# ddiazdom/grlBWT

Measured on AMD Instinct MI355X. Metric: input MB/s building BCR BWT on 10 GB DNA reads, 1/2/4/8 MI355X, higher is better.
Workload: dtype u8; 1 GPU; 66225166 x 150 bp Illumina-style reads (10000000066 bytes) from a 330000000 bp genome, 0.5% substitutions; BASELINE configs[3]; input_resident=HBM, output=.rl_bwt image in HBM, parallelism=1 GPU

## Files before the change

### grlbwt_amd/csrc/capi_impl.hpp

```cpp
#include "../../include/grlbwt_hip.h"

#include <fcntl.h>
#include <zlib.h>
#include <sys/stat.h>
#include <unistd.h>

#include <atomic>
#include <chrono>
#include <cstdio>
#include <cstring>
#include <condition_variable>
#include <memory>
#include <mutex>
#include <string>
#include <system_error>
#include <thread>
#include <vector>


struct grlbwt_fm {
    uint32_t flags = 0;
    std::unique_ptr<grl32::Engine::FmIndex> f32;
    std::unique_ptr<grl64::Engine::FmIndex> f64;
};
// ... 1360 lines not shown
    for (uint64_t nbits : sizes)
        for (int kind = 0; kind < 5; kind++) {
            if (int rc = test_set_bits_one<uint32_t>(nbits, kind, seed + kind)) return -(500 + rc);
            if (int rc = test_set_bits_one<uint64_t>(nbits, kind, seed + 7 + kind)) return -(510 + rc);
        }
#ifdef GRLBWT_PRIM_HIP
    for (uint32_t span = 8; span <= 64; span <<= 1)
        for (int kind = 2; kind <= 4; kind += 2) {
            if (int rc = test_set_bits_one<uint32_t>(sizes[6], kind, seed + 20 + kind, span)) return -(520 + rc);
            if (int rc = test_set_bits_one<uint64_t>(sizes[5], kind, seed + 30 + kind, span)) return -(530 + rc);
        }
#endif
    return 0;
}

int selftest(uint64_t n, uint64_t seed) {
    if (n < 2) n = 2;
    std::vector<uint32_t> h(n);
    uint64_t s = seed;
    for (uint64_t i = 0; i < n; i++) h[i] = (uint32_t)sm64(s);
    grl32::DBuf<uint32_t> d(n);
    prim::h2d(d.p, h.data(), n * 4);
    {
        grl32::DBuf<uint64_t> o(n + 1);
        uint64_t tot = prim::exclusive_scan<uint64_t>(n, U32In{d.p}, o.p, true, "selftest.scan");
        auto ho = o.to_host(n + 1);
        uint64_t acc = 0;
        for (uint64_t i = 0; i < n; i++) { if (ho[i] != acc) return -1; acc += h[i] & 1023u; }
        if (ho[n] != acc || tot != acc) return -2;
    }
// ... 44 lines not shown
    { int r = test_sort<uint64_t, uint32_t>(n, seed + 8, 51); if (r) return -110 - r; }
    { int r = test_sort_keys(n, seed + 9, 18); if (r) return -120 - r; }
    { int r = test_sort<uint32_t, uint64_t>(n, seed + 10, 27); if (r) return -130 - r; }
    { int r = test_sort<uint32_t, uint32_t>(n, seed + 11, 20); if (r) return -140 - r; }
    { int r = test_part(n, seed + 12, 6); if (r) return -150 - r; }
    { int r = test_part(n, seed + 13, 11); if (r) return -160 - r; }
    { int r = test_part(n, seed + 14, 18); if (r) return -170 - r; }
    { int r = test_pair_scan<uint32_t, uint32_t>(n, h, d.p); if (r) return -70 - r; }
    { int r = test_pair_scan<uint64_t, uint64_t>(n, h, d.p); if (r) return -80 - r; }
    { int r = test_stream_merge(n, seed); if (r) return r; }
#ifdef GRLBWT_PRIM_HIP
    { int r = test_seg_sort_all(seed + 40); if (r) return r; }
#endif
    { int r = test_pack(); if (r) return r; }
    { int r = test_set_bits(n, seed + 60); if (r) return r; }
    return 0;
}

}

extern "C" {

int grlbwt_abi_version(void) { return GRLBWT_ABI_VERSION; }
const char *grlbwt_backend_name(void) { return prim::kIsDevice ? "hip-gfx950" : "serial-test-standin"; }

const char *grlbwt_strerror(int code) {
    switch (code) {
        case GRLBWT_OK: return "ok";
        case GRLBWT_EINVAL: return "invalid argument or call out of order";
        case GRLBWT_EDEVICE: return "HIP device/runtime error";
// ... 555 lines not shown
```

### grlbwt_amd/csrc/engine_impl.hpp

```cpp

#include "switches.hpp"

namespace GRL_NS {

using prim::u8;
using prim::u16;
using prim::u32;
using prim::u64;
typedef GRL_IDX_T idx_t;

template <class T>
struct DBuf {
    T *p = nullptr;
    u64 n = 0;
    DBuf() {}
    explicit DBuf(u64 n_) { alloc(n_); }
    DBuf(const DBuf &) = delete;
    DBuf &operator=(const DBuf &) = delete;
    DBuf(DBuf &&o) noexcept : p(o.p), n(o.n) { o.p = nullptr; o.n = 0; }
    DBuf &operator=(DBuf &&o) noexcept {
        if (this != &o) { release(); p = o.p; n = o.n; o.p = nullptr; o.n = 0; }
        return *this;
    }
    ~DBuf() { release(); }
// ... 14 lines not shown
}

template <class T>
GRL_HD u64 upper_bound(const T *a, u64 n, T v) {
    u64 lo = 0, hi = n;
    while (lo < hi) { u64 mid = (lo + hi) >> 1; if (a[mid] <= v) lo = mid + 1; else hi = mid; }
    return lo;
}
template <class T>
GRL_HD u64 lower_bound(const T *a, u64 n, T v) {
    u64 lo = 0, hi = n;
    while (lo < hi) { u64 mid = (lo + hi) >> 1; if (a[mid] < v) lo = mid + 1; else hi = mid; }
    return lo;
}

template <class cell_t, bool FIRST>
struct CellOps {
    cell_t sep;
    GRL_HD u32 sym(cell_t c) const { return FIRST ? (u32)c : (u32)(c >> 2); }
    GRL_HD bool rep(cell_t c) const { return FIRST ? true : (bool)((c >> 1) & 1); }
    GRL_HD bool isT(cell_t c) const { return FIRST ? (c == sep) : (bool)(c & 1); }
};

GRL_HD bool bit_at(const u64 *w, u64 i) { return (w[i >> 6] >> (i & 63)) & 1ull; }
GRL_HD u64 next_set_bit(const u64 *w, u64 p, u64 n) {
    u64 r = n;
    if (p < n) {
        u64 wi = p >> 6;
        u64 x = w[wi] >> (p & 63);
        if (x) r = p + (u64)__builtin_ctzll(x);
        else {
            bool found = false;
            for (wi++; !found && (wi << 6) < n; wi++) { x = w[wi]; if (x) { r = (wi << 6) + (u64)__builtin_ctzll(x); found = true; } }
// ... 52 lines not shown
    const u64 *w;
    GRL_DEV u64 operator()(u64 i) const { return (u64)__builtin_popcountll(w[i]); }
};
struct PopcIn32 {
    const u64 *w;
    GRL_DEV u32 operator()(u64 i) const { return (u32)__builtin_popcountll(w[i]); }
};

static constexpr u64 kPosBits = 40;
static constexpr u64 kPosMask = (1ull << kPosBits) - 1;
static constexpr u64 kLenSat = 4095;
static constexpr u64 kExactKey = 1ull << 63;
GRL_HD u64 key_len(u64 k) { return (k >> kPosBits) & 0xFFFull; }
GRL_HD bool key_lastT(u64 k) { return (k >> (kPosBits + 12)) & 1ull; }
GRL_HD u64 key_pos(u64 k) { return (k & kPosMask) - 1; }

struct PhraseHash {
    u32 a, b;
    GRL_HD static PhraseHash init() { return PhraseHash{0x85A308D3u, 0x243F6A88u}; }
    GRL_HD void add(u32 v) {
        a = (a ^ v) * 0x9E3779B1u;
        b = (b + v) * 0x85EBCA6Bu;
        b ^= b >> 15;
    }
    GRL_HD u64 finish(u64 len) const {
        u64 h = ((u64)a << 32) | (u64)b;
        h ^= len * 0xC2B2AE3D27D4EB4Full;
        h ^= h >> 33; h *= 0xFF51AFD7ED558CCDull; h ^= h >> 33; h *= 0xC4CEB9FE1A85EC53ull; h ^= h >> 29;
        return h;
    }
// ... 42 lines not shown
    u64 hot_mask = 0;
    u32 slot_base = 0;
    static constexpr u32 kDirectSlots = 1u << 22;
    u32 dir_on = 0, dir_b0 = 0, dir_b1 = 0, dir_b2 = 0;
    u64 *dir_rep = nullptr;
    GRL_DEV u32 direct_index(u64 chunk, u32 len) const {
        const u64 ones = 0x0101010101010101ull;
        const u64 c = ((chunk >> dir_b0) & ones) | (((chunk >> dir_b1) & ones) << 1) | (((chunk >> dir_b2) & ones) << 2);
        const u32 lo = (u32)c, hi = (u32)(c >> 32);
        const u32 plo = (lo & 7u) | ((lo >> 5) & 0x38u) | ((lo >> 10) & 0x1C0u) | ((lo >> 15) & 0xE00u);
        const u32 phi = (hi & 7u) | ((hi >> 5) & 0x38u) | ((hi >> 10) & 0x1C0u) | ((hi >> 15) & 0xE00u);
        const u32 top = 1u << (3u * len);
        return ((plo | (phi << 12)) & (top - 1u)) | top;
    }
    GRL_DEV void first_seen(u32 slot, u64 item) const { if (dir_on && slot < kDirectSlots) dir_rep[slot] = item; }
    u64 *rec_k = nullptr; u64 *rec_hi = nullptr; int rec_b = 0; u32 rec_cmax = 0;
    u32 *long_count = nullptr;
    u64 walk_cap = ~0ull;
    static constexpr bool kExact = FIRST && sizeof(cell_t) == 1;
#ifndef GRL_HASH_BATCH
#define GRL_HASH_BATCH 4
#endif
    static constexpr int kBatch = kExact ? GRL_HASH_BATCH : 1;
    static constexpr u64 kCh = 8 / sizeof(cell_t);
    GRL_DEV static u64 load8(const cell_t *a) { u64 v; __builtin_memcpy(&v, a, 8); return v; }
    GRL_DEV bool same_phrase(u64 q, u64 p, u64 len, bool check_bits) const {
        bool same = true;
        if (q + len > n) { scal[1] = 3; scal[2] = (u32)q; scal[3] = (u32)len; same = false; }
        if (same && check_bits) {
            const u64 nq = next_set_bit(startbits, q + 1, n);
// ... 38 lines not shown
                const u64 len = (u64)eo + 1;
                if (ord >= n_occ) { scal[1] = 5; scal[2] = (u32)p; scal[3] = (u32)ord; }
                else if (rec_k) {
                    const u64 hi = khi | (((tm >> eo) & 1u) ? kPhrLastT : 0ull) | (len << 61);
                    rec_k[ord] = rec_key(klo, hi);
                    rec_hi[ord] = hi;
                    out_slot[ord] = 0;
                }
                fast = true;
            }
        }
        u32 res = prim::kNoBucket;
        if (!fast) res = process_walk(p, ord, pack);
        return res;
    }
    u64 *giant_list = nullptr; u32 *giant_n = nullptr; u32 giant_cap = 0;
    static constexpr u64 kLongWalk = 4096;
    GRL_DEV void giant_bounds(u64 item, u64 &p, u64 &ee) const {
        p = item;
        const u64 ns = next_set_bit_far(startbits, p + 1, n);
        ee = (ns >= n || ops.isT(t[ns - 1])) ? ns - 1 : ns;
    }
    GRL_DEV u64 giant_piece(u64 p, u64 ee, int lane) const {
        const u64 len = ee - p + 1, piece = (len + 63) / 64;
        u64 x = p + (u64)lane * piece;
        const u64 xe = x + piece < ee + 1 ? x + piece : ee + 1;
        const u64 cnt = xe > x ? xe - x : 0;
        PhraseHash ph = PhraseHash::init();
        while (x + 4 * kCh <= xe) {
            u64 ck[4];
// ... 83 lines not shown
                ok = false;
            } else {
                if (long_count) prim::atomic_add(long_count, 1u);
                if (rec_k) { rec_k[ord] = ord; rec_hi[ord] = 0ull; }
            }
        }
        if (ok) {
            u64 len = e - p + 1;
            if (kExact && len <= 7) {
                u64 content = 0;
                for (u64 j = 0; j < len; j++) content |= (u64)t[p + j] << (8 * j);
                const u64 mine = kExactKey | (len << 60) | content;
                if (dir_on) found = direct_index(content, (u32)len);
                else
                found = insert_exact(mine, p, exact_hash(mine) & (hot_keys ? hot_mask : mask), 0, false);
            } else found = find_or_insert(p, len, use_giant ? PhraseHash{(u32)(*giant_acc >> 32), (u32)*giant_acc}.finish(len) : ph.finish(len), ops.isT(t[e]));
            if (found != prim::kNoBucket) out_slot[ord] = (found & ~prim::kClaimBit) | (pack ? kLongMark : 0u);
        }
        return found;
    }
    GRL_DEV void process_batch(const u64 *item, const bool *valid, u32 *slot) const { process_batch_exact<false>(item, valid, slot, nullptr, nullptr); }
    static constexpr bool kStream = kExact;
    GRL_DEV u64 ordinal_base(u64 p) const { return (u64)wordbase[p >> 6]; }
    GRL_DEV u64 next_item(u64 p) const {
        const u64 b0 = p + 1;
        u64 bits = startbits[b0 >> 6] >> (b0 & 63);
        if ((b0 & 63) > 56) bits |= startbits[(b0 >> 6) + 1] << (64 - (b0 & 63));
        bits &= 0xFFull;
        return bits ? b0 + (u64)__builtin_ctzll(bits) : p + 9;
    }
// ... 272 lines not shown
    const u64 *words; const u32 *base; u64 *pos;
    GRL_DEV void operator()(u64 w) const {
        u64 x = words[w];
        u64 k = base[w];
        while (x) { pos[k++] = w * 64 + (u64)__builtin_ctzll(x); x &= x - 1; }
    }
};
template <class F>
struct ListedFn {
    F f; const u64 *pos;
    static constexpr int kBatch = 1;
    static constexpr bool kClaims = F::kClaims;
    u64 *claim_bits = nullptr;
    GRL_DEV u64 claim_pos(u64 v) const { return pos[v]; }
    GRL_DEV bool is_start(u64) const { return true; }
    GRL_DEV u32 process(u64 v) const { return f.process(pos[v]); }
    GRL_DEV u32 operator()(u64 v) const { return f.process(pos[v]); }
    GRL_DEV void process_batch(const u64 *, const bool *, u32 *) const {}
    GRL_DEV void first_seen(u32 slot, u64 v) const { f.first_seen(slot, pos[v]); }
};

template <class cell_t, bool FIRST>
struct CompactTableFn {
    const cell_t *t;
    CellOps<cell_t, FIRST> ops;
    const u64 *startbits;
    const u64 *keys; const idx_t *counts;
    u64 *ph_pos; idx_t *ph_freq; u32 *ph_len; u32 *ph_slot; u8 *ph_lastT;
    int ks; u64 cs; const u64 *rep_pos;
    u64 n;
    GRL_DEV void emit(u64 s, u64 k) const {
        u64 k64 = keys[s << ks];
        u64 pos, len;
        bool lastT;
        if (k64 & kExactKey) {
            len = (k64 >> 60) & 7ull;
            pos = rep_pos[s];
            lastT = ops.isT((cell_t)(k64 >> (8 * (len - 1))));
        } else {
            pos = key_pos(k64); len = key_len(k64);
            lastT = key_lastT(k64);
            if (len == kLenSat) {
                const u64 ns = next_set_bit_far(startbits, pos + 1, n);
                const u64 e = (ns >= n || ops.isT(t[ns - 1])) ? ns - 1 : ns;
                len = e - pos + 1;
            }
        }
        ph_pos[k] = pos; ph_freq[k] = counts[s * cs]; ph_len[k] = (u32)len; ph_slot[k] = (u32)s;
        ph_lastT[k] = lastT ? 1 : 0;
    }
// ... 2297 lines not shown
        u64 Ds = 0; int part_bits = 0, rec_b = 0; u32 slot0 = 0;
        DBuf<prim::U128> ph_key;
        DBuf<u32> lid, pbase;
        DBuf<u8> ph_vflag;
        DBuf<u64> pstart;
        prim::RecSort psort;
        void clear() {
            n_occ = D = S = cap = Ds = 0; maxlen = 0; part_bits = rec_b = 0; slot0 = 0;
            next_text.release(); ph_pos.release(); ph_freq.release(); ph_len.release(); ph_slot.release(); ph_off.release(); ph_lastT.release();
            ph_key.release(); ph_vflag.release(); pstart.release(); lid.release(); pbase.release(); psort.release();
        }
    };

    struct PartPlan { bool on = false; int rec_b = 0; u32 rec_cmax = 0; int part_bits = 0; };
    struct SamplePlan { u64 blk = 0, stride = 0, n = 0, distinct = 0, long_occ = 0; double frac = 1.0; };
    struct TablePlan { u64 cap = 0, cap_max = 0, cap_hot = 0; bool aggregate = false, interleaved = false, direct = false; int ks = 0; u64 cs = 1; u32 dir_b[3] = {0, 0, 0}; u64 sym_of_code = 0; };
    static bool direct_index_bits(const u64 sym_present[4], u32 bits[3], u64 &sym_of_code) {
        int syms[256], ns = 0;
        for (int i = 0; i < 256; i++) if ((sym_present[i >> 6] >> (i & 63)) & 1ull) syms[ns++] = i;
        if (ns > 8) return false;
        for (u32 a = 0; a < 8; a++) for (u32 b = a + 1; b < 8; b++) for (u32 c = b + 1; c < 8; c++) {
            u32 seen = 0; bool ok = true; u64 soc = 0;
            for (int k = 0; k < ns && ok; k++) {
                const u32 code = ((syms[k] >> a) & 1u) | (((syms[k] >> b) & 1u) << 1) | (((syms[k] >> c) & 1u) << 2);
                if (seen & (1u << code)) ok = false;
                seen |= 1u << code;
                soc |= (u64)syms[k] << (8 * code);
            }
            if (ok) { bits[0] = a; bits[1] = b; bits[2] = c; sym_of_code = soc; return true; }
        }
        return false;
// ... 59 lines not shown
            if (part.on) want = (u64)(3.0 * (double)smp.long_occ * ((double)n / (double)n_s)) + 4096;
            tab.cap = 4096; while (tab.cap < want) tab.cap <<= 1;
            if (tab.cap > tab.cap_max) tab.cap = tab.cap_max;
            if (prim::sw().table_trace) fprintf(stderr, "[grlbwt] level %d: sample %llu occurrences, %llu distinct -> table %llu slots for %llu occurrences\n",
                                                      prim::rt().tag, (unsigned long long)occ_s, (unsigned long long)smp.distinct, (unsigned long long)tab.cap, (unsigned long long)n_occ);
        }
        void plan_table() {
            claim.alloc(nwords + 1);
            if (part.on) { rec_k.alloc(n_occ); rec_hi.alloc(n_occ); }
            const bool force_direct = HF::kExact && !part.on && prim::sw().force_direct_index;
            tab.aggregate = smp.frac < 0.25 || force_direct;
            tab.interleaved = !tab.aggregate;
            tab.ks = tab.interleaved ? 1 : 0; tab.cs = tab.interleaved ? 16 / sizeof(idx_t) : 1;
            if (HF::kExact && tab.aggregate && (smp.n || force_direct) && !part.on && E.sym_present_known && !prim::sw().no_direct_index)
                tab.direct = direct_index_bits(E.sym_present, tab.dir_b, tab.sym_of_code);
            if (tab.direct && (const void *)t == E.text0 && E.text0 != (const void *)E.own0.p) {
                if constexpr (sizeof(cell_t) == 1) {
                    const u64 stride = n >= (1ull << 22) ? n >> 20 : 1, m = n / stride;
                    const u64 foreign = prim::reduce_sum<u64>(m, ForeignByteIn{(const u8 *)t, stride, E.sym_present[0], E.sym_present[1], E.sym_present[2], E.sym_present[3]}, "hash_prepare");
                    if (foreign) throw prim::Error(-22, "the attached text has changed since its statistics were taken (a cell value that was not there)");
                }
            }
            const bool hot = !tab.direct && tab.aggregate && smp.n && !part.on && !prim::sw().no_hot_table;
            if (!tab.direct && !hot) return;
            if (tab.direct) tab.cap_hot = HF::kDirectSlots;
            else for (tab.cap_hot = 1024; tab.cap_hot < 4 * smp.distinct;) tab.cap_hot <<= 1;
            if (tab.cap_max > (1ull << 30)) tab.cap_max = 1ull << 30;
            if (tab.cap > tab.cap_max) tab.cap = tab.cap_max;
            if (!prim::sw().table_trace) return;
            if (tab.direct) fprintf(stderr, "[grlbwt] level %d: direct index on bits %u, %u, %u of a cell (%llu slots in front of the table)\n", prim::rt().tag,
// ... 2 lines not shown
                         (unsigned long long)tab.cap_hot, (unsigned long long)smp.distinct);
        }
        void alloc_table() {
            if (tab.interleaved) { keys.alloc(2 * tab.cap); keys.zero(); }
            else { keys.alloc(tab.cap_hot + tab.cap); counts.alloc(tab.cap_hot + tab.cap); keys.zero(); counts.zero(); }
            cnt = tab.interleaved ? (idx_t *)(keys.p + 1) : counts.p;
            if (HF::kExact) rep_pos.alloc(tab.cap_hot + tab.cap);
            scal.zero(); claim.zero();
        }
        void fill_hot_table(HF &f) {
            HF fh{t, ops, startbits.p, wordbase.p, keys.p, tab.cap_hot - 1, tab.cap_hot, 0, P.next_text.p, scal.p, n, n_occ, rep_pos.p, claim.p};
            fh.walk_cap = HF::kLongWalk;
            prim::for_each_agg(smp.n, SampledFn<HF>{fh, smp.blk, smp.stride, claim.p}, NoCountAdd{}, false, "hash_hot");
            f.hot_keys = keys.p; f.hot_mask = tab.cap_hot - 1; f.slot_base = (u32)tab.cap_hot;
        }
        void hash_listed(const HF &f, DBuf<u64> &lbits, bool aggregate) {
            DBuf<u32> lbase(nwords + 1);
            const u64 nl = (u64)prim::exclusive_scan<u32>(nwords, PopcIn32{lbits.p}, lbase.p, false, "hash_long_list");
            DBuf<u64> lpos(nl ? nl : 1);
            if (nl) prim::for_each(nwords, BitPositionsFn{lbits.p, lbase.p, lpos.p}, "hash_long_list");
            lbits.release(); lbase.release();
            if (nl) prim::for_each_agg(nl, ListedFn<HF>{f, lpos.p, claim.p}, SlotCountAdd{cnt, tab.cs}, aggregate, "hash_long_phrases");
        }
        void records_and_long_phrases(const HF &f) {
            prim::dev_memset(P.next_text.p, 0, n_occ * sizeof(u32));
            DBuf<u64> lbits(nwords + 1); lbits.zero();
            auto records = [&](auto bw) {
                prim::for_each_set_bit<idx_t>(n, startbits.p, wordbase.p, PhraseRecordFn<cell_t, decltype(bw)::value>{t, ops, startbits.p, wordbase.p, n, n_occ,
                                                                                                               rec_k.p, rec_hi.p, part.rec_b, part.rec_cmax, lbits.p, scal.p}, "hash_phrases");
            };
            switch (part.rec_b) {
#define GRL_REC_CASE(BW) case BW: records(std::integral_constant<int, BW>()); break;
                GRL_REC_CASE(10) GRL_REC_CASE(11) GRL_REC_CASE(12) GRL_REC_CASE(13) GRL_REC_CASE(14) GRL_REC_CASE(15) GRL_REC_CASE(16)
// ... 3 lines not shown
                default: records(std::integral_constant<int, 0>()); break;
            }
            hash_listed(f, lbits, false);
        }
        void name_stream_and_long_phrases(const HF &f) {
            DBuf<u64> lbits(nwords + 1); lbits.zero();
            prim::name_stream(n, f, SlotCountAdd{cnt, tab.cs}, lbits.p, "hash_phrases");
            hash_listed(f, lbits, tab.aggregate);
        }
        bool hash_pass() {
            alloc_table();
            HF f{t, ops, startbits.p, wordbase.p, keys.p + tab.cap_hot, tab.cap - 1, (tab.cap == tab.cap_max) ? tab.cap : 96 , tab.ks,
                 P.next_text.p, scal.p, n, n_occ, rep_pos.p ? rep_pos.p + tab.cap_hot : nullptr, claim.p};
            if (part.on) { f.rec_k = rec_k.p; f.rec_hi = rec_hi.p; f.rec_b = part.rec_b; f.rec_cmax = part.rec_cmax; }
            f.giant_list = giant_list.p; f.giant_n = scal.p + 4; f.giant_cap = (u32)std::min<u64>(giant_cap, 0xFFFFFFFFull);
            if (tab.direct) { f.dir_on = 1; f.dir_b0 = tab.dir_b[0]; f.dir_b1 = tab.dir_b[1]; f.dir_b2 = tab.dir_b[2]; f.dir_rep = rep_pos.p; f.slot_base = (u32)tab.cap_hot; }
            else if (tab.cap_hot) fill_hot_table(f);
            if constexpr (!FIRST) {
                if (part.on && !prim::sw().part_one_pass) records_and_long_phrases(f);
                else prim::for_each_agg(n, f, SlotCountAdd{cnt, tab.cs}, tab.aggregate, "hash_phrases");
            } else if (tab.direct && n_occ < 0xFFFFFFF0ull && !prim::sw().no_name_stream) name_stream_and_long_phrases(f);
            else prim::for_each_agg(n, f, SlotCountAdd{cnt, tab.cs}, tab.aggregate, "hash_phrases");
            std::vector<u32> sc = scal.to_host(8);
            if (sc[4] && !sc[1]) {
                prim::for_each_giant((u64)sc[4], giant_list.p, f, SlotCountAdd{cnt, tab.cs}, "hash_giant_phrases");
                sc = scal.to_host(8);
            }
            if (sc[1] == 1) return false;
            if (sc[1]) throw prim::Error(-71, "phrase hashing: consistency check " + std::to_string(sc[1]) + " failed (" +
                                                   std::to_string(sc[2]) + ", " + std::to_string(sc[3]) + ")");
            if (tab.direct) prim::for_each(tab.cap_hot, DirectFixFn{cnt, keys.p, rep_pos.p, claim.p, tab.sym_of_code}, "hash_direct_fix");
            P.cap = tab.cap_hot + tab.cap;
            return true;
        }
        bool dedupe_partitions() {
            StageTimer st(&E.tm.hash, "hash");
            DBuf<u64> rec_k2(n_occ), rec_hi2(n_occ);
            const int res = P.psort.forward(rec_k.p, rec_hi.p, rec_k2.p, rec_hi2.p, n_occ, part.part_bits, "phrase_part");
            DBuf<u64> skey, shi;
            if (res) { skey = std::move(rec_k2); shi = std::move(rec_hi2); dkey = std::move(rec_k); dhi = std::move(rec_hi); }
            else { skey = std::move(rec_k); shi = std::move(rec_hi); dkey = std::move(rec_k2); dhi = std::move(rec_hi2); }
            const u64 nparts = (u64)1 << part.part_bits;
            P.pstart.alloc(nparts + 1);
            prim::for_each(nparts + 1, prim::RecBoundsFn{skey.p, n_occ, part.part_bits, nparts, P.pstart.p}, "phrase_part.bounds");
            P.lid.alloc(n_occ); P.pbase.alloc(nparts + 1); dcnt.alloc(n_occ);
// ... 15 lines not shown
            StageTimer st(&E.tm.dict_sort, "dict_sort");
            DBuf<idx_t> cbase(nwords + 1);
            const u64 Dl = (u64)prim::exclusive_scan<idx_t>(nwords, PopcIn{claim.p}, cbase.p, false, "table_compact");
            const u64 D = Ds + Dl;
            if (D >= 0xFFFFFFF0ull) throw prim::Error(-75, "dictionary too large (>= 2^32 phrases)");
            P.D = D;
            P.ph_pos.alloc(D); P.ph_freq.alloc(D); P.ph_len.alloc(D); P.ph_slot.alloc(D); P.ph_lastT.alloc(D); P.ph_off.alloc(D + 1);
            if (part.on) {
                P.ph_key.alloc(Ds); P.ph_vflag.alloc(Ds);
                prim::for_each(((u64)1 << part.part_bits) * 64, PartPhraseFn{P.pbase.p, P.pstart.p, dkey.p, dhi.p, dcnt.p, P.slot0, P.ph_key.p, P.ph_pos.p, P.ph_freq.p,
                                                                          P.ph_len.p, P.ph_slot.p, P.ph_lastT.p, P.ph_vflag.p}, "phrase_dedupe.phrases");
                dkey.release(); dhi.release(); dcnt.release();
            }
            prim::for_each(nwords, ClaimSlotsFn{claim.p, cbase.p, startbits.p, wordbase.p, P.next_text.p, P.ph_slot.p + Ds}, "table_compact");
            prim::for_each(Dl, ClaimCompactFn<cell_t, FIRST>{CompactTableFn<cell_t, FIRST>{t, ops, startbits.p, keys.p, cnt, P.ph_pos.p + Ds,
                                                             P.ph_freq.p + Ds, P.ph_len.p + Ds, P.ph_slot.p + Ds, P.ph_lastT.p + Ds, tab.ks, tab.cs, rep_pos.p, n}}, "table_compact");
            wordbase.release(); claim.release();
            const prim::Pair<u64, u64> fl = prim::reduce_sum<prim::Pair<u64, u64>>(D, FreqLenIn{P.ph_freq.p, P.ph_len.p}, "dict_totals");
            if (fl.a != n_occ) throw prim::Error(-71, "phrase frequencies (" + std::to_string(fl.a) + ") do not add up to the parse size (" +
                                                           std::to_string(n_occ) + ")");
            P.maxlen = prim::reduce_max<u32>(D, LenIn{P.ph_len.p}, "dict_maxlen");
            if (fl.b >= 0xFFFFFFF0ull) throw prim::Error(-75, "dictionary too large (>= 2^32 symbols)");
            prim::exclusive_scan_nosync<u32>(D, LenIn{P.ph_len.p}, P.ph_off.p, true, "dict_offsets");
            P.S = fl.b;
        }
    };
    template <class cell_t, bool FIRST>
    void hash_local(const cell_t *t, u64 n, CellOps<cell_t, FIRST> ops, LocalParse &P, LevelData &L, bool allow_part = false) {
        for (;; allow_part = false, P.clear()) {
            NameStage<cell_t, FIRST> Z(*this, t, n, ops, P, L);
            Z.classify();
// ... 2263 lines not shown
```

### grlbwt_amd/csrc/prim_hip.hpp

```cpp
#pragma once
#include <hip/hip_runtime.h>
#include <cstdint>
#include <cstdio>
#include <cstdlib>
#include <cstring>
#include <chrono>
#include <stdexcept>
#include <string>
#include <vector>
#include <map>
#include <utility>
#include <type_traits>

#define GRLBWT_PRIM_HIP 1
#include "switches.hpp"

#define GRL_HD __host__ __device__ __forceinline__
#define GRL_DEV __device__ __forceinline__

namespace prim {

typedef uint8_t u8;
typedef uint16_t u16;
typedef uint32_t u32;
// ... 581 lines not shown
        unsigned long long m = __ballot(b);
        if ((threadIdx.x & 63) == 0) words[i >> 6] = m;
    }
}
template <class F>
inline void bitvector_from_pred(u64 n, F pred, u64 *words, const char *name = "bitvector") {
    if (n == 0) return;
    u64 n_padded = (n + 63) & ~u64(63);
    prof_begin(name);
    hipLaunchKernelGGL(k_bitvector<F>, dim3(grid_for(n_padded, kBlock)), dim3(kBlock), 0, rt().stream, n_padded, n,
                       pred, words);
    prof_end();
    after_launch(name);
}

template <class cell_t, class OPS>
__global__ void __launch_bounds__(kBlock) k_start_bits(u64 n, const cell_t *t, OPS ops, u64 *words) {
    constexpr int CPL = 16 / (int)sizeof(cell_t);
    constexpr int TILE = kBlock * CPL;
    constexpr int C = sizeof(cell_t) == 1 ? 8 : (sizeof(cell_t) == 8 ? 2 : 4);
    constexpr int WPS = C;
    constexpr int STEP = 64 * C;
    struct alignas(16) Vec { cell_t v[CPL]; };
    __shared__ __attribute__((aligned(16))) cell_t s_raw[TILE + 2 * CPL];
    __shared__ __attribute__((aligned(8))) u8 s_m[kBlock / 64][4][8 * C];
    cell_t *s_c = s_raw + CPL;
    const int lane = threadIdx.x & 63, wave = threadIdx.x >> 6;
    const u64 ntiles = (n + TILE - 1) / TILE;
    const bool aligned = ((uintptr_t)t & 15) == 0;
    for (u64 tile = blockIdx.x; tile < ntiles; tile += gridDim.x) {
        const u64 base = tile * TILE;
        const u64 q0 = base + (u64)threadIdx.x * CPL;
        if (aligned && q0 + CPL <= n) {
            *reinterpret_cast<Vec *>(s_c + threadIdx.x * CPL) = *reinterpret_cast<const Vec *>(t + q0);
        } else {
#pragma unroll
            for (int k = 0; k < CPL; k++) s_c[threadIdx.x * CPL + k] = (q0 + k < n) ? t[q0 + k] : cell_t(0);
        }
        if (threadIdx.x == 0) s_c[-1] = base > 0 ? t[base - 1] : cell_t(0);
        if (threadIdx.x == 64) s_c[TILE] = (base + TILE < n) ? t[base + TILE] : cell_t(0);
        __syncthreads();
        for (int st = wave; st < TILE / STEP; st += kBlock / 64) {
            const int o = st * STEP + lane * C;
            const u64 p0 = base + (u64)o;
            cell_t c[C + 2];
#pragma unroll
            for (int j = 0; j < C + 2; j++) c[j] = s_c[o - 1 + j];
            u32 mg = 0, mp = 0, mf = 0, mc = 0;
#pragma unroll
            for (int j = 0; j < C; j++) {
                const u64 p = p0 + (u64)j;
                const bool in = p < n, has_nx = p + 1 < n;
                const cell_t cc = c[j + 1], nx = c[j + 2], pv = c[j];
                const u32 s = ops.sym(cc), sn = ops.sym(nx), sp = ops.sym(pv);
                const bool T = ops.isT(cc);
                if (in && has_nx && !T && sn > s) mg |= 1u << j;
                if (in && has_nx && !T && sn == s) mp |= 1u << j;
                if (in && (p == 0 || ops.isT(pv))) mf |= 1u << j;
                if (in && p > 0 && sp > s && ops.rep(pv) && ops.rep(cc)) mc |= 1u << j;
            }
#pragma unroll
            for (int k = C; k < 8; k *= 2) {
                mg |= (u32)__shfl_down((int)mg, k / C) << k;
                mp |= (u32)__shfl_down((int)mp, k / C) << k;
                mf |= (u32)__shfl_down((int)mf, k / C) << k;
                mc |= (u32)__shfl_down((int)mc, k / C) << k;
            }
            if (lane % (8 / C) == 0) {
                const int bi = lane / (8 / C);
                s_m[wave][0][bi] = (u8)mg; s_m[wave][1][bi] = (u8)mp; s_m[wave][2][bi] = (u8)mf; s_m[wave][3][bi] = (u8)mc;
            }
            __builtin_amdgcn_wave_barrier();
            if (lane < WPS) {
                const int wv = st * WPS + lane;
// ... 2782 lines not shown
```

### grlbwt_amd/csrc/switches.hpp

```cpp
#pragma once
#include <cstdint>
#include <cstdlib>

#define GRLBWT_SWITCHES_PRODUCT(X)                                                                                                 \
    X(GRLBWT_PART_MIN_OCC, part_min_occ, uint64_t, (uint64_t)1 << 20, "smallest level (phrase occurrences) that takes the partitioned naming") \
    X(GRLBWT_PART_BITS, part_bits, int, 0, "partition bits of the partitioned naming, 1..20 (0: from the level's size)")          \
    X(GRLBWT_PART_ONE_PASS, part_one_pass, bool, false, "partitioned naming: records and long phrases in one pass through the table") \
    X(GRLBWT_FORCE_DIRECT_INDEX, force_direct_index, bool, false, "take the direct index on texts too small for a sample")        \
    X(GRLBWT_TABLE_TRACE, table_trace, bool, false, "trace the phrase-table and cell-layout decisions on stderr")                 \
    X(GRLBWT_A2A_SELF_VIA_COMM, a2a_self_via_comm, bool, false, "a rank's own all-to-all block goes through the callback too")    \
    X(GRLBWT_RUN_KEYS_MIN, run_keys_min, uint64_t, 512, "phrase length from which the suffix sort takes run-aware keys")         \
    X(GRLBWT_DOUBLING_AFTER, doubling_after, uint64_t, 24, "refinement rounds of a long-phrase level before doubling rounds")     \
    X(GRLBWT_SEG_CAP, seg_cap, int, 64, "largest suffix group ordered by counting (kSegCap); larger ones in LDS or by two radix sorts") \
    X(GRLBWT_SEG_LDS_CAP, seg_lds_cap, int, 4096, "largest suffix group ordered in LDS (above: two radix sorts; 0: no LDS tier)") \
    X(GRLBWT_CELL_LAYOUT, cell_layout, char, 0, "p[acked] | s[eparate]: a wider induction cell layout than the input needs")     \
    X(GRLBWT_NO_CELL32, no_cell32, bool, false, "induction cells of one word in 64 bits even where 32 would do")               \
    X(GRLBWT_ASM_TWO_PASS, asm_two_pass, bool, false, "pass C always as count + emit (no one-walk form)")                       \
    X(GRLBWT_ASM_ONE_WALK, asm_one_walk, bool, false, "pass C tries the one-walk form at every level, plain or not")           \
    X(GRLBWT_ASM_IMAGE, asm_image, int, 1, "level 0's pass C writes the .rl_bwt records itself (0: emit + pack)")             \
    X(GRLBWT_DIST_GATHERED_DICT, dist_gathered_dict, bool, false, "multi-rank: the dictionary gathered on every rank, not sharded") \
    X(GRLBWT_DIST_SHARDED_DICT_MIN, dist_sharded_dict_min, int, 4, "multi-rank: ranks from which the dictionary is sharded")    \
    X(GRLBWT_DIST_SHARDED_DICT_MIN_SYMS, dist_sharded_dict_min_syms, uint64_t, (uint64_t)1 << 27, "multi-rank: dictionary symbols from which it is sharded") \
    X(GRLBWT_INVERT, invert, char, 0, "r[uns] | p[ositions]: the form of the inversion (unset: by the memory it needs)")         \
    X(GRLBWT_XS_MAXC, xs_maxc, int, 32, "most cells per item the fused expansion sort takes (lower: the unfused branch)")        \
    X(GRLBWT_ALPHA_TABLE_BITS, alpha_table_bits, int, 20, "log2 of the slots of the alphabet compaction's table, 2..26 (lower: the sorting regime)") \
    X(GRLBWT_FM_TOP_BITS, fm_top_bits, int, 12, "log2 of the keys of an FM index's search array kept in LDS, 0..12 (0: none; lower: small indexes search HBM)") \
    X(GRLBWT_IO_THREADS, io_threads, int, 0, "reader / writer threads per file chunk, 1..64 (0: from the host's cores)")         \
    X(GRLBWT_QUIET_ENV, quiet_env, bool, false, "no note on stderr about the switches set in the environment")

#define GRLBWT_SWITCHES_INIT(X)                                                                                                     \
    X(GRLBWT_TRACE, trace, char, 0, "1: print every launch and synchronise after it")                                          \
    X(GRLBWT_SYNC_SITES, sync_sites, bool, false, "profile: count behind which launch site the host waited")                  \
    X(GRLBWT_MEM_TRACE, mem_trace, bool, false, "per-stage peak device memory on stderr")                                      \
    X(GRLBWT_NOPOOL, nopool, bool, false, "no slab allocator: hipMalloc / hipFree for every buffer")                           \
// ... 104 lines not shown
```

Measured before the change: 13760 MB/s.

## Name 8-16 cell phrases by exact 3-bit coded keys and SWAR LMS typing

```diff
diff --git a/grlbwt_amd/csrc/capi_impl.hpp b/grlbwt_amd/csrc/capi_impl.hpp
--- a/grlbwt_amd/csrc/capi_impl.hpp
+++ b/grlbwt_amd/csrc/capi_impl.hpp
@@ -1398,6 +1398,75 @@
     return 0;
 }
 
+int test_lms_typing(uint64_t n, uint64_t seed) {
+    typedef grl32::CellOps<uint8_t, true> Ops;
+    static_assert(Ops::kPlainBytes && !grl32::CellOps<uint32_t, false>::kPlainBytes && !grl32::CellOps<uint16_t, true>::kPlainBytes, "the trait marks byte cells of level 0 only");
+    const int seps[3] = {0, 10, 255};
+    uint64_t s = seed;
+    for (int si = 0; si < 3; si++)
+        for (int a = 0; a < 256; a++)
+            for (int b = 0; b < 256; b++)
+                for (int j = -1; j < 8; j++) {
+                    uint8_t c[10];
+                    for (int k = 0; k < 10; k++) {
+                        const uint64_t r = sm64(s);
+                        c[k] = r % 5 == 0 ? (uint8_t)a : r % 5 == 1 ? (uint8_t)b : r % 5 == 2 ? (uint8_t)seps[si] : (uint8_t)(r >> 40);
+                    }
+                    c[j + 1] = (uint8_t)a; c[j + 2] = (uint8_t)b;
+                    uint64_t own = 0;
+                    for (int k = 0; k < 8; k++) own |= (uint64_t)c[k + 1] << (8 * k);
+                    uint32_t mg, mp, mf, mc, eg = 0, ep = 0, ef = 0, ec = 0;
+                    Ops{(uint8_t)seps[si]}.byte_masks((own << 8) | c[0], own, (own >> 8) | ((uint64_t)c[9] << 56), mg, mp, mf, mc);
+                    for (int k = 0; k < 8; k++) {
+                        const uint8_t cc = c[k + 1], nx = c[k + 2], pv = c[k];
+                        if (cc != seps[si] && nx > cc) eg |= 1u << k;
+                        if (cc != seps[si] && nx == cc) ep |= 1u << k;
+                        if (pv == seps[si]) ef |= 1u << k;
+                        if (pv > cc) ec |= 1u << k;
+                    }
+                    if (mg != eg || mp != ep || mf != ef || mc != ec) {
+                        fprintf(stderr, "[grlbwt] selftest lms masks: separator %d, cells %d %d at %d: G %02x/%02x P %02x/%02x first %02x/%02x cand %02x/%02x (got/expected)\n",
+                                seps[si], a, b, j, mg, eg, mp, ep, mf, ef, mc, ec);
+                        return -601;
+                    }
+                }
+    const uint64_t m = std::max<uint64_t>(self_size(n), 2);
+    for (int si = 0; si < 3; si++) {
+        const uint8_t sep = (uint8_t)seps[si];
+        std::vector<uint8_t> h(m + 1);
+        static const uint32_t runs[12] = {2, 2, 3, 3, 5, 8, 8, 20, 40, 70, 200, 3000};
+        for (uint64_t i = 0; i <= m;) {
+            const uint64_t r = sm64(s);
+            const uint8_t v = (uint8_t)(r >> 8);
+            for (uint64_t k = (r & 7) ? 1 : runs[(r >> 3) % 12]; k && i <= m; k--) h[i++] = v;
+        }
+        h[m - 1] = sep;
+        grl32::DBuf<uint8_t> d;
+        self_upload(d, h);
+        for (uint64_t off = 0; off < 2 && off + 2 <= m; off++) {
+            const uint64_t len = m - off, nw = (len + 63) / 64;
+            std::vector<uint8_t> t(h.begin() + off, h.begin() + off + len);
+            std::vector<uint8_t> S(len + 1, 0);
+            for (uint64_t q = len - 1; q-- > 0;) S[q] = t[q] != sep && (t[q + 1] > t[q] || (t[q + 1] == t[q] && S[q + 1]));
+            Ops ops{sep};
+            grl32::DBuf<uint64_t> w(nw + 1);
+            prim::dev_memset(w.p, 0xA5, (nw + 1) * 8);
+            prim::start_bitvector(len, (const uint8_t *)(d.p + off), ops, grl32::StartPred<uint8_t, true>{d.p + off, ops}, w.p, "selftest.start_bits");
+            const std::vector<uint64_t> hw = w.to_host(nw + 1);
+            for (uint64_t q = 0; q < nw * 64; q++) {
+                const bool want = q < len && (q == 0 || t[q - 1] == sep || (t[q - 1] > t[q] && S[q]));
+                if ((((hw[q >> 6] >> (q & 63)) & 1ull) != 0) != want) {
+                    fprintf(stderr, "[grlbwt] selftest start bits: %llu byte cells at offset %llu, separator %d: position %llu expected %d\n",
+                            (unsigned long long)len, (unsigned long long)off, seps[si], (unsigned long long)q, (int)want);
+                    return -602;
+                }
+            }
+            if (hw[nw] != 0xA5A5A5A5A5A5A5A5ull) return -603;
+        }
+    }
+    return 0;
+}
+
 int selftest(uint64_t n, uint64_t seed) {
     if (n < 2) n = 2;
     std::vector<uint32_t> h(n);
@@ -1472,6 +1541,7 @@
 #endif
     { int r = test_pack(); if (r) return r; }
     { int r = test_set_bits(n, seed + 60); if (r) return r; }
+    { int r = test_lms_typing(n, seed + 80); if (r) return r; }
     return 0;
 }
 
diff --git a/grlbwt_amd/csrc/engine_impl.hpp b/grlbwt_amd/csrc/engine_impl.hpp
--- a/grlbwt_amd/csrc/engine_impl.hpp
+++ b/grlbwt_amd/csrc/engine_impl.hpp
@@ -52,9 +52,42 @@
     return lo;
 }
 
+GRL_HD u32 lms_field_tops(u64 d) {
+#if defined(__HIP_DEVICE_COMPILE__)
+    return __builtin_amdgcn_perm((u32)(d >> 32), (u32)d, 0x07050301u);
+#else
+    return (u32)((d >> 8) & 0xFFull) | (u32)((d >> 16) & 0xFF00ull) | (u32)((d >> 24) & 0xFF0000ull) | (u32)((d >> 32) & 0xFF000000ull);
+#endif
+}
+GRL_HD u32 lms_merge8(u32 e, u32 o) {
+    u32 r = e | (o << 1);
+    r |= r >> 6;
+    r |= r >> 12;
+    return r & 0xFFu;
+}
+GRL_HD void lms_byte_masks(u64 pv, u64 own, u64 nx, u8 sep, u32 &mg, u32 &mp, u32 &mf, u32 &mc) {
+    const u64 M = 0x00FF00FF00FF00FFull, K = 0x0100010001000100ull, S = (u64)sep * 0x0001000100010001ull;
+    const u32 ONES = 0x01010101u;
+    const u64 xe = own & M, xo = (own >> 8) & M;
+    const u64 ze = pv & M, yo = (nx >> 8) & M;
+    const u32 ge_e = lms_field_tops((xe | K) - xo);
+    const u32 le_e = lms_field_tops((xo | K) - xe);
+    const u32 ge_o = lms_field_tops((xo | K) - yo);
+    const u32 le_o = lms_field_tops((yo | K) - xo);
+    const u32 gp_e = lms_field_tops((xe | K) - ze);
+    const u32 nt_e = lms_field_tops((xe ^ S) + M);
+    const u32 nt_o = lms_field_tops((xo ^ S) + M);
+    const u32 nt_z = lms_field_tops((ze ^ S) + M);
+    mg = lms_merge8(nt_e & (ge_e ^ ONES), nt_o & (ge_o ^ ONES));
+    mp = lms_merge8(nt_e & ge_e & le_e, nt_o & ge_o & le_o);
+    mf = lms_merge8(nt_z ^ ONES, nt_e ^ ONES);
+    mc = lms_merge8(gp_e ^ ONES, le_e ^ ONES);
+}
 template <class cell_t, bool FIRST>
 struct CellOps {
     cell_t sep;
+    static constexpr bool kPlainBytes = FIRST && sizeof(cell_t) == 1;
+    GRL_HD void byte_masks(u64 pv, u64 own, u64 nx, u32 &mg, u32 &mp, u32 &mf, u32 &mc) const { lms_byte_masks(pv, own, nx, (u8)sep, mg, mp, mf, mc); }
     GRL_HD u32 sym(cell_t c) const { return FIRST ? (u32)c : (u32)(c >> 2); }
     GRL_HD bool rep(cell_t c) const { return FIRST ? true : (bool)((c >> 1) & 1); }
     GRL_HD bool isT(cell_t c) const { return FIRST ? (c == sep) : (bool)(c & 1); }
@@ -137,6 +170,11 @@
 GRL_HD u64 key_len(u64 k) { return (k >> kPosBits) & 0xFFFull; }
 GRL_HD bool key_lastT(u64 k) { return (k >> (kPosBits + 12)) & 1ull; }
 GRL_HD u64 key_pos(u64 k) { return (k & kPosMask) - 1; }
+static constexpr u32 kCodedMin = 8, kCodedMax = 16;
+GRL_HD bool key_is_coded(u64 k) { return (k >> 60) == 8ull; }
+GRL_HD u64 coded_key(u64 codes, u32 len) { return kExactKey | ((u64)(len - kCodedMin) << 48) | (codes & ((1ull << (3u * len)) - 1ull)); }
+GRL_HD u32 coded_len(u64 k) { return kCodedMin + (u32)((k >> 48) & 15ull); }
+GRL_HD u32 coded_last(u64 k) { return (u32)(k >> (3u * (coded_len(k) - 1u))) & 7u; }
 
 struct PhraseHash {
     u32 a, b;
@@ -209,6 +247,16 @@
         return ((plo | (phi << 12)) & (top - 1u)) | top;
     }
     GRL_DEV void first_seen(u32 slot, u64 item) const { if (dir_on && slot < kDirectSlots) dir_rep[slot] = item; }
+    u32 long_exact = 0;
+    GRL_DEV u32 cell_codes(u64 chunk) const {
+        const u64 ones = 0x0101010101010101ull;
+        const u64 c = ((chunk >> dir_b0) & ones) | (((chunk >> dir_b1) & ones) << 1) | (((chunk >> dir_b2) & ones) << 2);
+        const u32 lo = (u32)c, hi = (u32)(c >> 32);
+        const u32 plo = (lo & 7u) | ((lo >> 5) & 0x38u) | ((lo >> 10) & 0x1C0u) | ((lo >> 15) & 0xE00u);
+        const u32 phi = (hi & 7u) | ((hi >> 5) & 0x38u) | ((hi >> 10) & 0x1C0u) | ((hi >> 15) & 0xE00u);
+        return plo | (phi << 12);
+    }
+    GRL_DEV u64 long_key(u64 c0, u64 c1, u32 len) const { return coded_key((u64)cell_codes(c0) | ((u64)cell_codes(c1) << 24), len); }
     u64 *rec_k = nullptr; u64 *rec_hi = nullptr; int rec_b = 0; u32 rec_cmax = 0;
     u32 *long_count = nullptr;
     u64 walk_cap = ~0ull;
@@ -277,6 +325,36 @@
         if (!fast) res = process_walk(p, ord, pack);
         return res;
     }
+    GRL_DEV u32 process_listed(u64 p) const {
+        u32 res = prim::kNoBucket;
+        bool lean = false;
+        if constexpr (kExact) {
+            if (dir_on && long_exact && p + 24 <= n) {
+                const u64 c0 = load8(t + p), c1 = load8(t + p + 8);
+                const u64 wi = p >> 6;
+                const u64 wp = startbits[wi], wn = startbits[wi + 1];
+                const u64 wb = (u64)wordbase[wi];
+                const u32 sh = (u32)(p & 63);
+                const u64 ord = wb + (u64)__builtin_popcountll(wp & ((1ull << sh) - 1ull));
+                const u32 sbits = (u32)(((wp >> sh) >> 1) | (wn << (63u - sh))) & 0xFFFFu;
+                const u32 spos = sbits ? (u32)__builtin_ctz(sbits) + 1u : 17u;
+                const u64 ones = 0x0101010101010101ull, sepx = (u64)ops.sep * ones;
+                const u64 x0 = c0 ^ sepx, x1 = c1 ^ sepx;
+                const u64 z0 = (x0 - ones) & ~x0 & (ones << 7), z1 = (x1 - ones) & ~x1 & (ones << 7);
+                const u32 tpos = z0 ? (u32)(__builtin_ctzll(z0) >> 3) : (z1 ? 8u + (u32)(__builtin_ctzll(z1) >> 3) : 16u);
+                const u32 len = (tpos < spos ? tpos : spos) + 1u;
+                lean = len >= kCodedMin && len <= kCodedMax;
+                if (lean) {
+                    const u64 mine = long_key(c0, c1, len);
+                    res = insert_exact(mine, p, exact_hash(mine) & mask, 0, false);
+                    if (ord >= n_occ) { scal[1] = 5; scal[2] = (u32)p; scal[3] = (u32)ord; res = prim::kNoBucket; }
+                    else if (res != prim::kNoBucket) out_slot[ord] = res & ~prim::kClaimBit;
+                }
+            }
+        }
+        if (!lean) res = process(p);
+        return res;
+    }
     u64 *giant_list = nullptr; u32 *giant_n = nullptr; u32 giant_cap = 0;
     static constexpr u64 kLongWalk = 4096;
     GRL_DEV void giant_bounds(u64 item, u64 &p, u64 &ee) const {
@@ -390,6 +468,15 @@
                 if (dir_on) found = direct_index(content, (u32)len);
                 else
                 found = insert_exact(mine, p, exact_hash(mine) & (hot_keys ? hot_mask : mask), 0, false);
+            } else if (kExact && dir_on && long_exact && len >= kCodedMin && len <= kCodedMax) {
+                u64 codes = 0;
+#pragma nounroll
+                for (u64 j = 0; j < len; j++) {
+                    const u32 c = (u32)t[p + j];
+                    codes |= (u64)(((c >> dir_b0) & 1u) | (((c >> dir_b1) & 1u) << 1) | (((c >> dir_b2) & 1u) << 2)) << (3 * j);
+                }
+                const u64 mine = coded_key(codes, (u32)len);
+                found = insert_exact(mine, p, exact_hash(mine) & mask, 0, false);
             } else found = find_or_insert(p, len, use_giant ? PhraseHash{(u32)(*giant_acc >> 32), (u32)*giant_acc}.finish(len) : ph.finish(len), ops.isT(t[e]));
             if (found != prim::kNoBucket) out_slot[ord] = (found & ~prim::kClaimBit) | (pack ? kLongMark : 0u);
         }
@@ -692,8 +779,8 @@
     u64 *claim_bits = nullptr;
     GRL_DEV u64 claim_pos(u64 v) const { return pos[v]; }
     GRL_DEV bool is_start(u64) const { return true; }
-    GRL_DEV u32 process(u64 v) const { return f.process(pos[v]); }
-    GRL_DEV u32 operator()(u64 v) const { return f.process(pos[v]); }
+    GRL_DEV u32 process(u64 v) const { return f.process_listed(pos[v]); }
+    GRL_DEV u32 operator()(u64 v) const { return f.process_listed(pos[v]); }
     GRL_DEV void process_batch(const u64 *, const bool *, u32 *) const {}
     GRL_DEV void first_seen(u32 slot, u64 v) const { f.first_seen(slot, pos[v]); }
 };
@@ -707,11 +794,16 @@
     u64 *ph_pos; idx_t *ph_freq; u32 *ph_len; u32 *ph_slot; u8 *ph_lastT;
     int ks; u64 cs; const u64 *rep_pos;
     u64 n;
+    u32 sep_code = 8;
     GRL_DEV void emit(u64 s, u64 k) const {
         u64 k64 = keys[s << ks];
         u64 pos, len;
         bool lastT;
-        if (k64 & kExactKey) {
+        if (key_is_coded(k64)) {
+            len = coded_len(k64);
+            pos = rep_pos[s];
+            lastT = coded_last(k64) == sep_code;
+        } else if (k64 & kExactKey) {
             len = (k64 >> 60) & 7ull;
             pos = rep_pos[s];
             lastT = ops.isT((cell_t)(k64 >> (8 * (len - 1))));
@@ -3039,7 +3131,8 @@
 
     struct PartPlan { bool on = false; int rec_b = 0; u32 rec_cmax = 0; int part_bits = 0; };
     struct SamplePlan { u64 blk = 0, stride = 0, n = 0, distinct = 0, long_occ = 0; double frac = 1.0; };
-    struct TablePlan { u64 cap = 0, cap_max = 0, cap_hot = 0; bool aggregate = false, interleaved = false, direct = false; int ks = 0; u64 cs = 1; u32 dir_b[3] = {0, 0, 0}; u64 sym_of_code = 0; };
+    struct TablePlan { u64 cap = 0, cap_max = 0, cap_hot = 0; bool aggregate = false, interleaved = false, direct = false; int ks = 0; u64 cs = 1; u32 dir_b[3] = {0, 0, 0}; u64 sym_of_code = 0;
+                       u32 sep_code = 8; };
     static bool direct_index_bits(const u64 sym_present[4], u32 bits[3], u64 &sym_of_code) {
         int syms[256], ns = 0;
         for (int i = 0; i < 256; i++) if ((sym_present[i >> 6] >> (i & 63)) & 1ull) syms[ns++] = i;
@@ -3129,6 +3222,10 @@
             tab.ks = tab.interleaved ? 1 : 0; tab.cs = tab.interleaved ? 16 / sizeof(idx_t) : 1;
             if (HF::kExact && tab.aggregate && (smp.n || force_direct) && !part.on && E.sym_present_known && !prim::sw().no_direct_index)
                 tab.direct = direct_index_bits(E.sym_present, tab.dir_b, tab.sym_of_code);
+            if (tab.direct) {
+                const u32 sp = (u32)ops.sep & 0xFFu;
+                if ((E.sym_present[sp >> 6] >> (sp & 63)) & 1ull) tab.sep_code = ((sp >> tab.dir_b[0]) & 1u) | (((sp >> tab.dir_b[1]) & 1u) << 1) | (((sp >> tab.dir_b[2]) & 1u) << 2);
+            }
             if (tab.direct && (const void *)t == E.text0 && E.text0 != (const void *)E.own0.p) {
                 if constexpr (sizeof(cell_t) == 1) {
                     const u64 stride = n >= (1ull << 22) ? n >> 20 : 1, m = n / stride;
@@ -3161,9 +3258,21 @@
             prim::for_each_agg(smp.n, SampledFn<HF>{fh, smp.blk, smp.stride, claim.p}, NoCountAdd{}, false, "hash_hot");
             f.hot_keys = keys.p; f.hot_mask = tab.cap_hot - 1; f.slot_base = (u32)tab.cap_hot;
         }
+        u64 listed = 0;
+        void trace_long_phrases() {
+            const std::vector<u64> hk = keys.to_host(tab.cap_hot + tab.cap);
+            const std::vector<idx_t> hc = counts.to_host(tab.cap_hot + tab.cap);
+            u64 dc = 0, oc = 0, dg = 0, og = 0;
+            for (u64 s = tab.cap_hot; s < tab.cap_hot + tab.cap; s++)
+                if (hk[s]) { if (key_is_coded(hk[s])) { dc++; oc += (u64)hc[s]; } else { dg++; og += (u64)hc[s]; } }
+            fprintf(stderr, "[grlbwt] level %d: %llu of %llu phrase occurrences listed (more than 7 cells, or the last cells of the text); the table holds %llu coded keys "
+                            "(8..16 cells) with %llu occurrences and %llu other phrases with %llu\n", prim::rt().tag, (unsigned long long)listed, (unsigned long long)n_occ,
+                    (unsigned long long)dc, (unsigned long long)oc, (unsigned long long)dg, (unsigned long long)og);
+        }
         void hash_listed(const HF &f, DBuf<u64> &lbits, bool aggregate) {
             DBuf<u32> lbase(nwords + 1);
             const u64 nl = (u64)prim::exclusive_scan<u32>(nwords, PopcIn32{lbits.p}, lbase.p, false, "hash_long_list");
+            listed = nl;
             DBuf<u64> lpos(nl ? nl : 1);
             if (nl) prim::for_each(nwords, BitPositionsFn{lbits.p, lbase.p, lpos.p}, "hash_long_list");
             lbits.release(); lbase.release();
@@ -3197,7 +3306,10 @@
                  P.next_text.p, scal.p, n, n_occ, rep_pos.p ? rep_pos.p + tab.cap_hot : nullptr, claim.p};
             if (part.on) { f.rec_k = rec_k.p; f.rec_hi = rec_hi.p; f.rec_b = part.rec_b; f.rec_cmax = part.rec_cmax; }
             f.giant_list = giant_list.p; f.giant_n = scal.p + 4; f.giant_cap = (u32)std::min<u64>(giant_cap, 0xFFFFFFFFull);
-            if (tab.direct) { f.dir_on = 1; f.dir_b0 = tab.dir_b[0]; f.dir_b1 = tab.dir_b[1]; f.dir_b2 = tab.dir_b[2]; f.dir_rep = rep_pos.p; f.slot_base = (u32)tab.cap_hot; }
+            if (tab.direct) {
+                f.dir_on = 1; f.dir_b0 = tab.dir_b[0]; f.dir_b1 = tab.dir_b[1]; f.dir_b2 = tab.dir_b[2]; f.dir_rep = rep_pos.p; f.slot_base = (u32)tab.cap_hot;
+                f.long_exact = prim::sw().name_long_exact != 0 ? 1u : 0u;
+            }
             else if (tab.cap_hot) fill_hot_table(f);
             if constexpr (!FIRST) {
                 if (part.on && !prim::sw().part_one_pass) records_and_long_phrases(f);
@@ -3212,6 +3324,7 @@
             if (sc[1] == 1) return false;
             if (sc[1]) throw prim::Error(-71, "phrase hashing: consistency check " + std::to_string(sc[1]) + " failed (" +
                                                    std::to_string(sc[2]) + ", " + std::to_string(sc[3]) + ")");
+            if (tab.direct && prim::sw().table_trace) trace_long_phrases();
             if (tab.direct) prim::for_each(tab.cap_hot, DirectFixFn{cnt, keys.p, rep_pos.p, claim.p, tab.sym_of_code}, "hash_direct_fix");
             P.cap = tab.cap_hot + tab.cap;
             return true;
@@ -3257,7 +3370,7 @@
             }
             prim::for_each(nwords, ClaimSlotsFn{claim.p, cbase.p, startbits.p, wordbase.p, P.next_text.p, P.ph_slot.p + Ds}, "table_compact");
             prim::for_each(Dl, ClaimCompactFn<cell_t, FIRST>{CompactTableFn<cell_t, FIRST>{t, ops, startbits.p, keys.p, cnt, P.ph_pos.p + Ds,
-                                                             P.ph_freq.p + Ds, P.ph_len.p + Ds, P.ph_slot.p + Ds, P.ph_lastT.p + Ds, tab.ks, tab.cs, rep_pos.p, n}}, "table_compact");
+                                                             P.ph_freq.p + Ds, P.ph_len.p + Ds, P.ph_slot.p + Ds, P.ph_lastT.p + Ds, tab.ks, tab.cs, rep_pos.p, n, tab.sep_code}}, "table_compact");
             wordbase.release(); claim.release();
             const prim::Pair<u64, u64> fl = prim::reduce_sum<prim::Pair<u64, u64>>(D, FreqLenIn{P.ph_freq.p, P.ph_len.p}, "dict_totals");
             if (fl.a != n_occ) throw prim::Error(-71, "phrase frequencies (" + std::to_string(fl.a) + ") do not add up to the parse size (" +
diff --git a/grlbwt_amd/csrc/prim_hip.hpp b/grlbwt_amd/csrc/prim_hip.hpp
--- a/grlbwt_amd/csrc/prim_hip.hpp
+++ b/grlbwt_amd/csrc/prim_hip.hpp
@@ -619,6 +619,10 @@
     after_launch(name);
 }
 
+template <class OPS>
+constexpr auto ops_plain_bytes(int) -> decltype(OPS::kPlainBytes) { return OPS::kPlainBytes; }
+template <class OPS>
+constexpr bool ops_plain_bytes(long) { return false; }
 template <class cell_t, class OPS>
 __global__ void __launch_bounds__(kBlock) k_start_bits(u64 n, const cell_t *t, OPS ops, u64 *words) {
     constexpr int CPL = 16 / (int)sizeof(cell_t);
@@ -648,10 +652,21 @@
         for (int st = wave; st < TILE / STEP; st += kBlock / 64) {
             const int o = st * STEP + lane * C;
             const u64 p0 = base + (u64)o;
+            u32 mg = 0, mp = 0, mf = 0, mc = 0;
+            if constexpr (ops_plain_bytes<OPS>(0)) {
+                static_assert(C == 8, "eight byte cells per lane");
+                const u64 own = *reinterpret_cast<const u64 *>(s_c + o);
+                const u64 pv = (own << 8) | (u64)s_c[o - 1], nx = (own >> 8) | ((u64)s_c[o + 8] << 56);
+                ops.byte_masks(pv, own, nx, mg, mp, mf, mc);
+                const u64 left = p0 < n ? n - p0 : 0;
+                const u32 inm = left >= 8 ? 0xFFu : (1u << (u32)left) - 1u;
+                const u32 nxm = left >= 9 ? 0xFFu : (left ? (1u << (u32)(left - 1)) - 1u : 0u);
+                mg &= nxm; mp &= nxm; mf &= inm; mc &= inm;
+                if (p0 == 0) { mf |= inm & 1u; mc &= ~1u; }
+            } else {
             cell_t c[C + 2];
 #pragma unroll
             for (int j = 0; j < C + 2; j++) c[j] = s_c[o - 1 + j];
-            u32 mg = 0, mp = 0, mf = 0, mc = 0;
 #pragma unroll
             for (int j = 0; j < C; j++) {
                 const u64 p = p0 + (u64)j;
@@ -663,6 +678,7 @@
                 if (in && has_nx && !T && sn == s) mp |= 1u << j;
                 if (in && (p == 0 || ops.isT(pv))) mf |= 1u << j;
                 if (in && p > 0 && sp > s && ops.rep(pv) && ops.rep(cc)) mc |= 1u << j;
+            }
             }
 #pragma unroll
             for (int k = C; k < 8; k *= 2) {
diff --git a/grlbwt_amd/csrc/switches.hpp b/grlbwt_amd/csrc/switches.hpp
--- a/grlbwt_amd/csrc/switches.hpp
+++ b/grlbwt_amd/csrc/switches.hpp
@@ -18,6 +18,7 @@
     X(GRLBWT_ASM_TWO_PASS, asm_two_pass, bool, false, "pass C always as count + emit (no one-walk form)")                       \
     X(GRLBWT_ASM_ONE_WALK, asm_one_walk, bool, false, "pass C tries the one-walk form at every level, plain or not")           \
     X(GRLBWT_ASM_IMAGE, asm_image, int, 1, "level 0's pass C writes the .rl_bwt records itself (0: emit + pack)")             \
+    X(GRLBWT_NAME_LONG_EXACT, name_long_exact, int, 1, "level 0 with the direct index: phrases of 8..16 cells by exact coded keys (0: hashed, the walk)") \
     X(GRLBWT_DIST_GATHERED_DICT, dist_gathered_dict, bool, false, "multi-rank: the dictionary gathered on every rank, not sharded") \
     X(GRLBWT_DIST_SHARDED_DICT_MIN, dist_sharded_dict_min, int, 4, "multi-rank: ranks from which the dictionary is sharded")    \
     X(GRLBWT_DIST_SHARDED_DICT_MIN_SYMS, dist_sharded_dict_min_syms, uint64_t, (uint64_t)1 << 27, "multi-rank: dictionary symbols from which it is sharded") \
```

Result: no change. 13800 MB/s (median of 6 runs) (+0.3%).
